# uibk-uncover/ws-unet

Measured on AMD Instinct MI355X. Metric: 512x512 grayscale images/sec (UNet predict), higher is better.
Workload: dtype f16 MFMA on the f16 halves + ONE block-scaled fp4 (e2m1) MFMA per tap pair for both residual cross terms (per-pixel / per-(co, tap) E8M0 scales), fp32 accumulate; planar storage

## Files before the change

### ws_unet_amd/csrc/conv3x3_qu.hip

```cpp
#include "wsu_device.h"

namespace {

constexpr int TW = 32, TH = 16;
constexpr int CW = 17, CH = 9, CPIX = CW * CH;
constexpr int NPIX_S = 4 * CPIX;
constexpr int PLANE_S = NPIX_S * 16;
constexpr int SEG_S = (NPIX_S + 63) / 64;
constexpr int IN_S = 3 * PLANE_S + SEG_S * 256;
constexpr int LP = 33, LH = TH / 2 + 2, LW_ = TW / 2 + 2;
constexpr int NPIX_L = LP * LH;
constexpr int PLANE_L = NPIX_L * 16;
constexpr int SEG_L = (NPIX_L + 63) / 64;
constexpr int IN_L = 3 * PLANE_L + SEG_L * 256;
constexpr int W_GRAN_S = 9 * 3 * WSU_COB * 16;
constexpr int W_S = W_GRAN_S + 1024;
constexpr int W_UNITS_L = 8;
constexpr int W_GRAN_L = W_UNITS_L * 3 * WSU_COB * 16;
constexpr int W_L = W_GRAN_L + 1024;
constexpr int PIECES_S = W_S / 1024, PIECES_L = W_L / 1024;
constexpr int REGION = 80640;
constexpr int OFF_SW = IN_S, OFF_LIN = W_L, OFF_LW1 = W_L + IN_L;
constexpr int LDS_BIAS = 2 * REGION;
constexpr int MAX_COUT = 512;
constexpr int LDS_TOTAL = LDS_BIAS + MAX_COUT * 4;
static_assert(IN_S + W_S <= REGION && OFF_LW1 + W_L <= REGION && (REGION & 0xF) == 0 && LDS_TOTAL <= 160 * 1024, "LDS budget");
static_assert((OFF_SW | OFF_LIN | OFF_LW1) % 16 == 0, "16-byte aligned allocations");
constexpr int ZERO_BYTES = 576;
constexpr int LDS_ZERO = 2 * REGION - ZERO_BYTES;
static_assert(IN_S + W_S <= REGION - ZERO_BYTES && OFF_LW1 + W_L <= REGION - ZERO_BYTES && LDS_ZERO % 16 == 0 && ZERO_BYTES >= 2 * CW * 16 + 16 + 16, "zero block");
constexpr int NLOAD = 4, NWAVE = 8, NT = (NWAVE + NLOAD) * 64;
constexpr unsigned OOB = 0xFFFFFFF0u;
constexpr int W_S_H = 9 * 2 * WSU_COB * 16;
constexpr int W_L_H = W_UNITS_L * 2 * WSU_COB * 16;
constexpr int PIECES_S_H = W_S_H / 1024, PIECES_L_H = W_L_H / 1024;

struct UArgs {
    const char* xl; const char* xs; const char* wps; const char* wpl; const float* bias;
    char* y;
    int n, h, w, hl, wl, cl, c2, cout;
    int tiles_x, tiles_y, ltiles_x, ncb, nchS, nchL;
    int relu, ntiles;
    unsigned* range_flag;
};

struct Tile { int n, y0, x0, cb; };
__device__ __forceinline__ Tile tile_of(const UArgs& a, int t) {
    Tile r;
    r.cb = t % a.ncb; t /= a.ncb;
    const int tx = t % a.tiles_x; t /= a.tiles_x;
    const int ty = t % a.tiles_y;
    r.n = t / a.tiles_y; r.y0 = ty * TH; r.x0 = tx * TW;
    return r;
}

typedef __attribute__((address_space(3))) void lds_void;
typedef __attribute__((address_space(3))) char lds_char;

__device__ __forceinline__ void wait_vm(int n) {
#define WSU_VM_CASE(k) case k: asm volatile("s_waitcnt vmcnt(" #k ")" ::: "memory"); break;
    switch (n) {
        WSU_VM_CASE(0) WSU_VM_CASE(1) WSU_VM_CASE(2) WSU_VM_CASE(3) WSU_VM_CASE(4) WSU_VM_CASE(5) WSU_VM_CASE(6) WSU_VM_CASE(7) WSU_VM_CASE(8) WSU_VM_CASE(9)
        WSU_VM_CASE(10) WSU_VM_CASE(11) WSU_VM_CASE(12) WSU_VM_CASE(13) WSU_VM_CASE(14) WSU_VM_CASE(15) WSU_VM_CASE(16) WSU_VM_CASE(17) WSU_VM_CASE(18) WSU_VM_CASE(19)
        WSU_VM_CASE(20) WSU_VM_CASE(21) WSU_VM_CASE(22) WSU_VM_CASE(23) WSU_VM_CASE(24) WSU_VM_CASE(25) WSU_VM_CASE(26) WSU_VM_CASE(27) WSU_VM_CASE(28) WSU_VM_CASE(29)
        WSU_VM_CASE(30) WSU_VM_CASE(31) WSU_VM_CASE(32) WSU_VM_CASE(33) WSU_VM_CASE(34) WSU_VM_CASE(35) WSU_VM_CASE(36) WSU_VM_CASE(37) WSU_VM_CASE(38) WSU_VM_CASE(39)
        default: asm volatile("s_waitcnt vmcnt(0)" ::: "memory"); break;
    }
#undef WSU_VM_CASE
}


template <int FMT, int LW>
__device__ __forceinline__ void u_loader(const UArgs& a, char* smem, int lane, int lw, int G, int K) {
    constexpr bool H = FMT == WSU_PLANAR_H;
    constexpr int NSS = LW < 2 ? 3 : 2;
    constexpr int NSL = LW < 2 ? 2 : 1;
    constexpr int OPS_INS = (H ? 2 : 4) * NSS, OPS_INL = (H ? 2 : 4) * NSL;
    constexpr int WS0 = H ? (LW < 2 ? LW * 3 : 6 + (LW - 2) * 6) : (LW < 2 ? LW * 5 : 10 + (LW - 2) * 9);
    constexpr int NWS = H ? (LW < 2 ? 3 : 6) : (LW < 2 ? 5 : 9);
    constexpr int WL0 = H ? (LW < 2 ? LW * 3 : 6 + (LW - 2) * 5) : (LW < 2 ? LW * 5 : (LW == 2 ? 10 : 17));
    constexpr int NWL = H ? (LW < 2 ? 3 : 5) : (LW < 2 ? 5 : (LW == 2 ? 7 : 8));
    constexpr int WSLICE_S = H ? W_S_H : W_S, WSLICE_L = H ? W_L_H : W_L;
    static_assert(2 * 5 + 2 * 9 == PIECES_S && 2 * 5 + 7 + 8 == PIECES_L, "weight pieces over the loader waves");
    static_assert(2 * 3 + 2 * 6 == PIECES_S_H && 2 * 3 + 2 * 5 == PIECES_L_H, "weight pieces over the loader waves (format H)");
    lds_char* smem3 = (lds_char*)smem;
    const unsigned hw16 = (unsigned)(a.h * a.w) * 16u, hwl16 = (unsigned)(a.hl * a.wl) * 16u;
    const unsigned cbytes_s = H ? (unsigned)wsu_h_chunk_bytes(a.h, a.w) : (unsigned)wsu_q_chunk_bytes(a.h, a.w);
    const unsigned cbytes_l = H ? (unsigned)wsu_h_chunk_bytes(a.hl, a.wl) : (unsigned)wsu_q_chunk_bytes(a.hl, a.wl);
    const int T = a.nchS + a.nchL;
    const int J = K * T;
    if (J <= 0) return;
    unsigned voS[NSS], soS[NSS], voL[NSL], soL[NSL];
    auto plan = [&](const Tile& t) __attribute__((always_inline)) {
        WSU_STATIC_FOR(NSS, k, {
            const int idx = min((LW + NLOAD * k) * 64 + lane, NPIX_S - 1);
            const int p = idx / CPIX, rem = idx - p * CPIX;
            const int lr = rem / CW, lc = rem - lr * CW;
            const int yy = wsu_reflect(t.y0 - 1 + 2 * lr + (p >> 1), a.h), xx = wsu_reflect(t.x0 - 1 + 2 * lc + (p & 1), a.w);
            voS[k] = (unsigned)(yy * a.w + xx) * 16u;
            if constexpr (!H) soS[k] = 3u * hw16 + wsu_q_soff(yy, xx, a.tiles_x);
        });
        WSU_STATIC_FOR(NSL, k, {
            const int idx = min((LW + NLOAD * k) * 64 + lane, NPIX_L - 1);
            const int r = idx / LP, c = min(idx - r * LP, LW_ - 1);
            const int yy = min(max((t.y0 >> 1) - 1 + r, 0), a.hl - 1), xx = min(max((t.x0 >> 1) - 1 + c, 0), a.wl - 1);
            voL[k] = (unsigned)(yy * a.wl + xx) * 16u;
            if constexpr (!H) soL[k] = 3u * hwl16 + wsu_q_soff(yy, xx, a.ltiles_x);
        });
    };
    int a_kt = 0, a_c = 0, a_r = 0; bool a_low = false;
    Tile at = tile_of(a, lw);
    unsigned region = 0;
    auto issue_alloc = [&](lds_char* slot) __attribute__((always_inline)) {
        int nops;
        const bool is_in = a_low ? a_r == 1 : a_r == 0;
        if (is_in && !a_low) {
            const char* src = a.xs + ((size_t)at.n * a.nchS + a_c) * cbytes_s;
            const auto rs = __builtin_amdgcn_make_buffer_rsrc(const_cast<char*>(src), 0, (int)cbytes_s, 0x00020000);
            WSU_STATIC_FOR(NSS, k, {
                constexpr int seg = LW + NLOAD * k;
                if (seg < SEG_S - 1 || lane < NPIX_S - (SEG_S - 1) * 64) {
                    __builtin_amdgcn_raw_ptr_buffer_load_lds(rs, (lds_void*)(slot + seg * 1024), 16, voS[k], 0, 0, 0);
                    __builtin_amdgcn_raw_ptr_buffer_load_lds(rs, (lds_void*)(slot + PLANE_S + seg * 1024), 16, voS[k], (int)hw16, 0, 0);
                    if constexpr (!H) {
                        __builtin_amdgcn_raw_ptr_buffer_load_lds(rs, (lds_void*)(slot + 2 * PLANE_S + seg * 1024), 16, voS[k], (int)(2u * hw16), 0, 0);
                        __builtin_amdgcn_raw_ptr_buffer_load_lds(rs, (lds_void*)(slot + 3 * PLANE_S + seg * 256), 1, soS[k], 0, 0, 0);
                    }
                }
            });
            nops = OPS_INS;
        } else if (is_in) {
            const char* src = a.xl + ((size_t)at.n * a.nchL + a_c) * cbytes_l;
            const auto rs = __builtin_amdgcn_make_buffer_rsrc(const_cast<char*>(src), 0, (int)cbytes_l, 0x00020000);
            WSU_STATIC_FOR(NSL, k, {
                constexpr int seg = LW + NLOAD * k;
                if (seg < SEG_L - 1 || lane < NPIX_L - (SEG_L - 1) * 64) {
                    __builtin_amdgcn_raw_ptr_buffer_load_lds(rs, (lds_void*)(slot + seg * 1024), 16, voL[k], 0, 0, 0);
                    __builtin_amdgcn_raw_ptr_buffer_load_lds(rs, (lds_void*)(slot + PLANE_L + seg * 1024), 16, voL[k], (int)hwl16, 0, 0);
                    if constexpr (!H) {
                        __builtin_amdgcn_raw_ptr_buffer_load_lds(rs, (lds_void*)(slot + 2 * PLANE_L + seg * 1024), 16, voL[k], (int)(2u * hwl16), 0, 0);
                        __builtin_amdgcn_raw_ptr_buffer_load_lds(rs, (lds_void*)(slot + 3 * PLANE_L + seg * 256), 1, soL[k], 0, 0, 0);
                    }
                }
            });
            nops = OPS_INL;
        } else if (!a_low) {
            const auto rs = __builtin_amdgcn_make_buffer_rsrc(const_cast<char*>(a.wps), 0, 0x7FFFFFF0, 0x00020000);
            const int base = (at.cb * a.nchS + a_c) * WSLICE_S;
            WSU_STATIC_FOR(NWS, k, {
                constexpr int piece = WS0 + k;
                __builtin_amdgcn_raw_ptr_buffer_load_lds(rs, (lds_void*)(slot + piece * 1024), 16, (unsigned)lane * 16u, base + piece * 1024, 0, 0);
            });
            nops = NWS;
        } else {
            const auto rs = __builtin_amdgcn_make_buffer_rsrc(const_cast<char*>(a.wpl), 0, 0x7FFFFFF0, 0x00020000);
            const int base = ((at.cb * a.nchL + a_c) * 2 + (a_r == 2 ? 1 : 0)) * WSLICE_L;
            WSU_STATIC_FOR(NWL, k, {
                constexpr int piece = WL0 + k;
                __builtin_amdgcn_raw_ptr_buffer_load_lds(rs, (lds_void*)(slot + piece * 1024), 16, (unsigned)lane * 16u, base + piece * 1024, 0, 0);
            });
            nops = NWL;
        }
        return nops;
    };
    auto issue_step = [&]() __attribute__((always_inline)) {
        lds_char* base = smem3 + region;
        int nops;
        if (!a_low) {
            a_r = 0; nops = issue_alloc(base);
            a_r = 1; nops += issue_alloc(base + OFF_SW);
            if (++a_c == a.nchS) { a_c = 0; a_low = true; }
        } else {
            a_r = 0; nops = issue_alloc(base);
            a_r = 1; nops += issue_alloc(base + OFF_LIN);
            a_r = 2; nops += issue_alloc(base + OFF_LW1);
            if (++a_c == a.nchL) {
                a_low = false; a_c = 0;
                if (++a_kt < K) { at = tile_of(a, lw + a_kt * G); plan(at); }
            }
        }
        region ^= (unsigned)REGION;
        return nops;
    };
    plan(at);
    {
        issue_step();
        const int n1 = J > 1 ? issue_step() : 0;
        wait_vm(n1);
    }
    for (int j = 0; ; ++j) {
        __builtin_amdgcn_s_barrier();
        asm volatile("" ::: "memory");
        if (j + 1 >= J) break;
        if (j >= 1) issue_step();
        wait_vm(0);
    }
}

template <int FMT>
__global__ __launch_bounds__(NT) __attribute__((amdgpu_waves_per_eu(3, 3)))
void conv3x3_qu_kernel(const UArgs a) {
    constexpr bool H = FMT == WSU_PLANAR_H;
    constexpr int WPL = H ? 2 : 3;
    extern __shared__ __attribute__((aligned(16))) char smem[];
    const int tid = threadIdx.x;
    const int wv = __builtin_amdgcn_readfirstlane(tid >> 6), lane = tid & 63;
    const int G = gridDim.x;
    const int lw = (int)wsu_xcd_remap(blockIdx.x, G);
    const int K = a.ntiles > lw ? (a.ntiles - lw + G - 1) / G : 0;
    float* s_bias = reinterpret_cast<float*>(smem + LDS_BIAS);
    for (int i = tid; i < a.cout; i += NT) s_bias[i] = a.bias ? a.bias[i] : 0.f;
    if constexpr (!H) {
        for (int i = tid; i < ZERO_BYTES / 4; i += NT) reinterpret_cast<unsigned*>(smem + LDS_ZERO)[i] = 0u;
        asm volatile("s_waitcnt lgkmcnt(0)" ::: "memory");
    }

    if (wv >= NWAVE) {
        switch (wv - NWAVE) {
            case 0: u_loader<FMT, 0>(a, smem, lane, lw, G, K); break;
            case 1: u_loader<FMT, 1>(a, smem, lane, lw, G, K); break;
            case 2: u_loader<FMT, 2>(a, smem, lane, lw, G, K); break;
            default: u_loader<FMT, 3>(a, smem, lane, lw, G, K); break;
        }
        return;
    }

    const int cls = wv & 3, py = cls >> 1, px = cls & 1, rh = wv >> 2;
    const int l31 = lane & 31, hh = lane >> 5;
    const int lrow = l31 >> 4, lcol = lrow ? ((l31 + 15) & 15) : l31;
    const unsigned laneS = (unsigned)(((4 * rh + lrow) * CW + lcol) * 16), laneL = (unsigned)(((4 * rh + lrow) * LP + lcol) * 16);
    constexpr unsigned QS = 2 * CW * 16, QL = 2 * LP * 16;
    Tile cur = tile_of(a, lw);
    f32x16 acc[2][2];
    unsigned region = 0;
    unsigned in_off = 0, w_off = 0;
    auto next_region = [&]() __attribute__((always_inline)) { const unsigned r = region; region ^= (unsigned)REGION; return r; };
    int hh_q = hh;
    typedef __attribute__((address_space(3))) const unsigned char lds_cuchar;
    typedef __attribute__((address_space(3))) const int lds_cint;
    typedef __attribute__((address_space(3))) const u32x4 lds_cu32x4;
    lds_char* L = (lds_char*)smem;
    const unsigned Lb = (unsigned)(size_t)L;
    auto at = [](unsigned addr) __attribute__((always_inline)) { return (lds_char*)(size_t)addr; };
    auto tap_s = [&](int ky, int kx) __attribute__((always_inline)) {
        return (unsigned)(((((py + ky) & 1) * 2 + ((px + kx) & 1)) * CPIX + ((py + ky) >> 1) * CW + ((px + kx) >> 1)) * 16);
    };
    unsigned a_off = 0, b_off = 0, hd_w = 0, hd_sa = 0, hd_b = 0, hd_sb = 0, x_w = 0, x_w4 = 0, x_sa = 0, x_sa4 = 0, x_b4 = 0;
    constexpr unsigned W4_IMM = (unsigned)((8 * 3 + 2) * 64) * 16u;
    unsigned tap_sel[5] = {};
    if constexpr (!H) {
        WSU_STATIC_FOR(5, tp, {
            constexpr int t0 = 2 * tp, t1 = (2 * tp + 1 < 9) ? 2 * tp + 1 : 2 * tp;
            tap_sel[tp] = ((hh ? tap_s(t1 / 3, t1 % 3) : tap_s(t0 / 3, t0 % 3)) + laneS) >> 2;
            asm volatile("" : "+v"(tap_sel[tp]));
        });
    }
    auto sync_step = [&](auto low_c) __attribute__((always_inline)) {
        constexpr bool LOW = decltype(low_c)::value;
        const unsigned r = next_region();
        in_off = LOW ? r + OFF_LIN : r;
        w_off = LOW ? r : r + OFF_SW;
        hh_q = hh;
        asm volatile("" : "+v"(hh_q));
        a_off = Lb + w_off + (unsigned)l31 * 16u + (unsigned)hh * 1024u;
        b_off = Lb + in_off + (unsigned)hh * (LOW ? PLANE_L : PLANE_S) + (LOW ? laneL : laneS);
        if constexpr (!H && !LOW) {
            const unsigned hq = (unsigned)hh_q, zero = Lb + (unsigned)LDS_ZERO;
            const unsigned w0 = Lb + w_off + (unsigned)l31 * 16u;
            x_w = w0 + hq * (unsigned)(3 * 64 * 16);
            x_w4 = hq ? zero - W4_IMM : w0;
            x_sa4 = Lb + w_off + W_GRAN_S + (unsigned)l31;
            x_sa = x_sa4 + hq * 64u;
            hd_b = Lb + in_off + 2 * PLANE_S + tap_sel[0] * 4u;
            hd_sb = Lb + in_off + 3 * PLANE_S + tap_sel[0];
            x_b4 = hq ? zero : Lb + in_off + 2 * PLANE_S + tap_sel[4] * 4u;
            asm volatile("" : "+v"(a_off), "+v"(b_off), "+v"(x_w), "+v"(x_w4), "+v"(x_sa), "+v"(x_sa4), "+v"(hd_b), "+v"(hd_sb), "+v"(x_b4));
        } else if constexpr (!H) {
            const int u = cls * 2 + hh_q;
            const unsigned pb = (unsigned)((py * LP + px) * 16) + (unsigned)hh_q * 16u + laneL;
            hd_w = Lb + w_off + (unsigned)((u * 3 + 2) * 64 + l31) * 16u;
            hd_sa = Lb + w_off + W_GRAN_L + (unsigned)(u * 64 + l31);
            hd_b = Lb + in_off + 2 * PLANE_L + pb;
            hd_sb = Lb + in_off + 3 * PLANE_L + (pb >> 2);
            asm volatile("" : "+v"(a_off), "+v"(b_off), "+v"(hd_w), "+v"(hd_sa), "+v"(hd_b), "+v"(hd_sb));
        } else {
            asm volatile("" : "+v"(a_off), "+v"(b_off));
        }
        __builtin_amdgcn_s_barrier();
        asm volatile("" ::: "memory");
    };
    struct Frag { u32x4 a[2]; u32x4 b[2]; int sa[2]; int sb[2]; };
    auto load_unit = [&](auto u_c, Frag& f) __attribute__((always_inline)) {
        constexpr int u = decltype(u_c)::value, tp = u / 3, k = u % 3;
        if constexpr (k == 0) {
            constexpr bool single = 2 * tp + 1 >= 9;
            constexpr unsigned wimm = (unsigned)((6 * tp + 2) * 64) * 16u;
            static_assert(!single || wimm == W4_IMM, "tap 8");
            const unsigned wb = single ? x_w4 : x_w, sab = single ? x_sa4 : x_sa;
            const unsigned bb = tp == 0 ? hd_b : (single ? x_b4 : Lb + in_off + 2 * PLANE_S + tap_sel[tp] * 4u);
            const unsigned sbb = tp == 0 ? hd_sb : Lb + in_off + 3 * PLANE_S + tap_sel[tp];
_Pragma("unroll")
            for (int m = 0; m < 2; ++m) { f.a[m] = *(lds_cu32x4*)(at(wb) + wimm + m * 512); f.sa[m] = *(lds_cuchar*)(at(sab) + 128 * tp + m * 32); }
_Pragma("unroll")
            for (int q = 0; q < 2; ++q) {
                f.b[q] = *(lds_cu32x4*)(at(bb) + q * QS);
                f.sb[q] = *(lds_cint*)(at(sbb) + q * (QS >> 2));
            }
        } else {
            constexpr int tap = 2 * tp + k - 1;
            const unsigned pb = b_off + tap_s(tap / 3, tap % 3);
_Pragma("unroll")
            for (int m = 0; m < 2; ++m) f.a[m] = *(lds_cu32x4*)(at(a_off) + ((tap * WPL) * 64) * 16 + m * 512);
_Pragma("unroll")
            for (int q = 0; q < 2; ++q) f.b[q] = *(lds_cu32x4*)(at(pb) + q * QS);
        }
    };
    auto mma_unit = [&](auto u_c, Frag& f, auto first_c) __attribute__((always_inline)) {
        constexpr int u = decltype(u_c)::value, k = u % 3;
        constexpr bool FIRST = decltype(first_c)::value && u == 0;
_Pragma("unroll")
        for (int m = 0; m < 2; ++m)
_Pragma("unroll")
            for (int q = 0; q < 2; ++q) {
                if constexpr (k != 0) wsu_mfma_f16(f.a[m], f.b[q], acc[m][q]);
                else if constexpr (FIRST) acc[m][q] = wsu_mfma_q4_z(f.a[m], f.b[q], f.sa[m], f.sb[q]);
                else wsu_mfma_q4(f.a[m], f.b[q], f.sa[m], f.sb[q], acc[m][q]);
            }
    };
    auto skip_units = [&](auto first_c) __attribute__((always_inline)) {
        constexpr bool FIRST = decltype(first_c)::value;
        if constexpr (!H) {
            constexpr int NU = 14;
            Frag fr[2];
            load_unit(std::integral_constant<int, 0>{}, fr[0]);
            WSU_STATIC_FOR(NU, u, {
                if constexpr (u + 1 < NU) load_unit(std::integral_constant<int, u + 1>{}, fr[(u + 1) % 2]);
                __builtin_amdgcn_sched_barrier(0);
                mma_unit(u_c, fr[u % 2], first_c);
                __builtin_amdgcn_sched_barrier(0);
            });
        } else {
            WSU_STATIC_FOR(9, tap, {
                u32x4 ah[2], bh[2];
                const unsigned pb = b_off + tap_s(tap / 3, tap % 3);
_Pragma("unroll")
                for (int m = 0; m < 2; ++m) ah[m] = *(lds_cu32x4*)(at(a_off) + ((tap * WPL) * 64) * 16 + m * 512);
_Pragma("unroll")
                for (int q = 0; q < 2; ++q) bh[q] = *(lds_cu32x4*)(at(pb) + q * QS);
_Pragma("unroll")
                for (int m = 0; m < 2; ++m)
_Pragma("unroll")
                    for (int q = 0; q < 2; ++q) {
                        if constexpr (FIRST && tap == 0) acc[m][q] = wsu_mfma_f16_z(ah[m], bh[q]);
                        else wsu_mfma_f16(ah[m], bh[q], acc[m][q]);
                    }
            });
        }
    };
    auto low_units = [&](auto dy_c) __attribute__((always_inline)) {
        constexpr int dy = decltype(dy_c)::value;
        constexpr unsigned WDY = dy ? (unsigned)(OFF_LW1) : 0u;
        const unsigned rowo = (unsigned)(((py + dy) * LP + px) * 16);
        if constexpr (!H) {
            const int u = cls * 2 + hh_q;
            u32x4 a4[2], b4[2]; int sa[2], sb[2];
            const unsigned pb = rowo + (unsigned)hh_q * 16u + laneL;
            const unsigned wb = dy == 0 ? hd_w : Lb + w_off + WDY + (unsigned)((u * 3 + 2) * 64 + l31) * 16u;
            const unsigned sab = dy == 0 ? hd_sa : Lb + w_off + WDY + W_GRAN_L + (unsigned)(u * 64 + l31);
            const unsigned bb = dy == 0 ? hd_b : Lb + in_off + 2 * PLANE_L + pb;
            const unsigned sbb = dy == 0 ? hd_sb : Lb + in_off + 3 * PLANE_L + (pb >> 2);
_Pragma("unroll")
            for (int m = 0; m < 2; ++m) { a4[m] = *(lds_cu32x4*)(at(wb) + m * 512); sa[m] = *(lds_cuchar*)(at(sab) + m * 32); }
_Pragma("unroll")
            for (int q = 0; q < 2; ++q) {
                b4[q] = *(lds_cu32x4*)(at(bb) + q * QL);
                sb[q] = *(lds_cint*)(at(sbb) + q * (QL >> 2));
            }
_Pragma("unroll")
            for (int m = 0; m < 2; ++m)
_Pragma("unroll")
                for (int q = 0; q < 2; ++q) wsu_mfma_q4(a4[m], b4[q], sa[m], sb[q], acc[m][q]);
        }
        WSU_STATIC_FOR(2, dx, {
            u32x4 ah[2], bh[2];
            const unsigned wb = a_off + WDY + (unsigned)(((cls * 2 + dx) * WPL) * 64) * 16u;
            const unsigned pb = b_off + rowo + dx * 16u;
_Pragma("unroll")
            for (int m = 0; m < 2; ++m) ah[m] = *(lds_cu32x4*)(at(wb) + m * 512);
_Pragma("unroll")
            for (int q = 0; q < 2; ++q) bh[q] = *(lds_cu32x4*)(at(pb) + q * QL);
_Pragma("unroll")
            for (int m = 0; m < 2; ++m)
_Pragma("unroll")
                for (int q = 0; q < 2; ++q) wsu_mfma_f16(ah[m], bh[q], acc[m][q]);
        });
    };

    auto finish_tile = [&]() __attribute__((always_inline)) {
        int l31o = l31, hho = hh, lro = lrow, lco = lcol;
        asm volatile("" : "+v"(l31o), "+v"(hho), "+v"(lro), "+v"(lco));
        const unsigned hw16 = (unsigned)(a.h * a.w) * 16u;
        const unsigned cbytes = (unsigned)wsu_q_chunk_bytes(a.h, a.w);
        const int nco = a.cout >> 4;
        const int X = cur.x0 + 2 * lco + px;
        const int Y0 = cur.y0 + 2 * (4 * rh + lro) + py, Y1 = Y0 + 4;
        const bool ok0 = Y0 < a.h && X < a.w, ok1 = Y1 < a.h && X < a.w;
        const unsigned off0 = (unsigned)(Y0 * a.w + X) * 16u, off1 = (unsigned)(Y1 * a.w + X) * 16u;
        const unsigned so0 = wsu_q_soff(Y0, X, a.tiles_x), so1 = wsu_q_soff(Y1, X, a.tiles_x);
        const unsigned hpl = hho ? hw16 : 0u;
        const bool okm = hho ? ok1 : ok0;
        unsigned og0 = ok0 ? off0 + hpl : OOB, og1 = ok1 ? off1 + hpl : OOB;
        unsigned oq = okm ? (hho ? off1 : off0) + 2u * hw16 : OOB, os = okm ? 3u * hw16 + (hho ? so1 : so0) : OOB;
        asm volatile("" : "+v"(og0), "+v"(og1), "+v"(oq), "+v"(os));
        const float relu_floor = a.relu ? 0.f : -__builtin_inff();
        float vmax = 0.f;
        WSU_STATIC_FOR(2, m, {
            WSU_STATIC_FOR(2, cp, {
                const int oc = cur.cb * 4 + m * 2 + cp;
                const int co0 = oc * 16 + 4 * hho;
                const f32x4 bx = *reinterpret_cast<const f32x4*>(s_bias + co0), by = *reinterpret_cast<const f32x4*>(s_bias + co0 + 8);
                f32x4 vx[2], vy[2];
_Pragma("unroll")
                for (int q = 0; q < 2; ++q)
_Pragma("unroll")
                    for (int e = 0; e < 4; ++e) {
                        const float x = fmaxf(acc[m][q][8 * cp + e] + bx[e], relu_floor), y = fmaxf(acc[m][q][8 * cp + 4 + e] + by[e], relu_floor);
                        vx[q][e] = x; vy[q][e] = y;
                        if constexpr (H) vmax = fmaxf(fmaxf(vmax, fabsf(x)), fabsf(y));
                    }
                if constexpr (H) {
                    char* base = a.y + ((size_t)cur.n * nco + oc) * (2u * hw16);
                    const auto rs = __builtin_amdgcn_make_buffer_rsrc(base, 0, (int)(2u * hw16), 0x00020000);
                    __builtin_amdgcn_raw_buffer_store_b128(wsu_h_granule(vx[0], vy[0]), rs, (int)og0, 0, 0);
                    __builtin_amdgcn_raw_buffer_store_b128(wsu_h_granule(vx[1], vy[1]), rs, (int)og1, 0, 0);
                    return;
                }
                u32x4 g0, g1; uint32_t dh0, dr0, sb0, dh1, dr1, sb1;
                const float mx0 = wsu_q4_pre(vx[0], vy[0], g0, dh0, dr0, sb0);
                const float mx1 = wsu_q4_pre(vx[1], vy[1], g1, dh1, dr1, sb1);
                vmax = wsu_max3(vmax, mx0, mx1);
                const u32x4 qg = wsu_q4_pair(dh0, dr0, dh1, dr1);
                char* base = a.y + ((size_t)cur.n * nco + oc) * cbytes;
                const auto rs = __builtin_amdgcn_make_buffer_rsrc(base, 0, (int)cbytes, 0x00020000);
                __builtin_amdgcn_raw_buffer_store_b128(g0, rs, (int)og0, 0, 0);
                __builtin_amdgcn_raw_buffer_store_b128(g1, rs, (int)og1, 0, 0);
                __builtin_amdgcn_raw_buffer_store_b128(qg, rs, (int)oq, 0, 0);
                __builtin_amdgcn_raw_buffer_store_b8((unsigned char)(hho ? sb1 : sb0), rs, (int)os, 0, 0);
            });
        });
        if (a.range_flag && __builtin_amdgcn_ballot_w64(!(vmax <= (H ? WSU_F16_RANGE : WSU_F8_RANGE))) != 0 && lane == 0) atomicOr(a.range_flag, 1u);
    };

    for (int t = 0; t < K; ++t) {
        sync_step(std::false_type{});
        skip_units(std::true_type{});
        for (int c = 1; c < a.nchS; ++c) {
            sync_step(std::false_type{});
            skip_units(std::false_type{});
        }
        for (int c = 0; c < a.nchL; ++c) {
            sync_step(std::true_type{});
            low_units(std::integral_constant<int, 0>{});
            low_units(std::integral_constant<int, 1>{});
        }
        finish_tile();
        if (t + 1 < K) cur = tile_of(a, lw + (t + 1) * G);
    }
}

template <int FMT>
__global__ void pack_up_low_kernel(const float* __restrict__ w3, const float* __restrict__ wt, char* __restrict__ dst, float* __restrict__ wc_dense,
                                   int cup, int c2, int cl, int cout) {
    const int nchL = cl / 16, ctot = cup + c2;
    const long long total = (long long)(cout / WSU_COB) * nchL * 2 * W_UNITS_L * WSU_COB;
    for (long long d = (long long)blockIdx.x * blockDim.x + threadIdx.x; d < total; d += (long long)gridDim.x * blockDim.x) {
        long long t = d;
        const int co = (int)(t % WSU_COB); t /= WSU_COB;
        const int u = (int)(t % W_UNITS_L); t /= W_UNITS_L;
        const int dy = (int)(t & 1); t >>= 1;
        const int c = (int)(t % nchL); const int cb = (int)(t / nchL);
        const int cls = u >> 1, dx = u & 1, py = cls >> 1, px = cls & 1;
        const int ky0 = py == 0 ? (dy == 0 ? 0 : 1) : (dy == 0 ? 0 : 2), ky1 = py == 0 ? (dy == 0 ? 0 : 2) : (dy == 0 ? 1 : 2);
        const int kx0 = px == 0 ? (dx == 0 ? 0 : 1) : (dx == 0 ? 0 : 2), kx1 = px == 0 ? (dx == 0 ? 0 : 2) : (dx == 0 ? 1 : 2);
        const int cog = cb * WSU_COB + co;
        float v[16], r[16];
#pragma unroll
        for (int e = 0; e < 16; ++e) v[e] = 0.f;
        for (int ci = 0; ci < cup; ++ci)
            for (int ky = ky0; ky <= ky1; ++ky)
                for (int kx = kx0; kx <= kx1; ++kx) {
                    const float w = w3[(((size_t)cog * ctot + ci) * 3 + ky) * 3 + kx];
                    const int sy = (py + ky + 1) & 1, sx = (px + kx + 1) & 1;
#pragma unroll
                    for (int e = 0; e < 16; ++e) v[e] = fmaf(w, wt[(((size_t)(c * 16 + e) * cup + ci) * 2 + sy) * 2 + sx], v[e]);
                }
        if (wc_dense)
#pragma unroll
            for (int e = 0; e < 16; ++e) wc_dense[((((size_t)cog * cl + c * 16 + e) * 2 + py) * 2 + px) * 4 + dy * 2 + dx] = v[e];
        uint32_t h[8];
#pragma unroll
        for (int e = 0; e < 8; ++e) {
            const _Float16 x = (_Float16)v[2 * e], y = (_Float16)v[2 * e + 1];
            h[e] = (uint32_t)__builtin_bit_cast(unsigned short, x) | ((uint32_t)__builtin_bit_cast(unsigned short, y) << 16);
            r[2 * e] = (v[2 * e] - (float)x) * 2048.f; r[2 * e + 1] = (v[2 * e + 1] - (float)y) * 2048.f;
        }
        const u32x4 h0 = mk_u4(h[0], h[1], h[2], h[3]), h1 = mk_u4(h[4], h[5], h[6], h[7]);
        if constexpr (FMT == WSU_PLANAR_H) {
            char* base = dst + (((size_t)cb * nchL + c) * 2 + dy) * W_L_H + (size_t)(u * 2) * (WSU_COB * 16) + co * 16;
            *reinterpret_cast<u32x4*>(base) = h0;
            *reinterpret_cast<u32x4*>(base + WSU_COB * 16) = h1;
            continue;
        }
        const int E = wsu_q4_block_exp(wsu_f16x16_max_abs_bits(h0, h1));
        const float sc = wsu_pow2f(E);
        uint32_t q[4] = {0, 0, 0, 0};
        WSU_STATIC_FOR(8, e, { q[e >> 2] = __builtin_amdgcn_cvt_scalef32_pk_fp4_f32(q[e >> 2], r[2 * e], r[2 * e + 1], sc, e & 3); });
        q[2] = wsu_f16x8_to_fp4(h0, sc); q[3] = wsu_f16x8_to_fp4(h1, sc);
        char* slice = dst + (((size_t)cb * nchL + c) * 2 + dy) * W_L;
        char* base = slice + (size_t)(u * 3) * (WSU_COB * 16) + co * 16;
        *reinterpret_cast<u32x4*>(base) = h0;
        *reinterpret_cast<u32x4*>(base + WSU_COB * 16) = h1;
        *reinterpret_cast<u32x4*>(base + 2 * WSU_COB * 16) = mk_u4(q[0], q[1], q[2], q[3]);
        slice[W_GRAN_L + u * 64 + co] = (char)(E + 127 - 11);
        if (u == 0 && co < 32) *reinterpret_cast<u32x4*>(slice + W_GRAN_L + 512 + co * 16) = mk_u4(0, 0, 0, 0);
    }
}

__global__ void up_bias_kernel(const float* __restrict__ w3, const float* __restrict__ bt, const float* __restrict__ b3, float* __restrict__ out, int cup, int c2, int cout) {
    const int co = blockIdx.x * blockDim.x + threadIdx.x;
    if (co >= cout) return;
    float s = b3 ? b3[co] : 0.f;
    if (bt)
        for (int ci = 0; ci < cup; ++ci) {
            float t = 0.f;
            for (int k = 0; k < 9; ++k) t += w3[((size_t)co * (cup + c2) + ci) * 9 + k];
            s = fmaf(bt[ci], t, s);
        }
    out[co] = s;
}

struct UFormat {
    const char* pack; const char* fwd;
    void (*pack_kernel)(const float*, const float*, char*, float*, int, int, int, int); const char* pack_kernel_name;
    void (*kernel)(const UArgs); const char* kernel_name; const char* lds_name;
    int w_s, w_l;
};
const UFormat& u_format(int fmt) {
    static const UFormat q = {"conv3x3_up_pack", "conv3x3_up_q", pack_up_low_kernel<WSU_PLANAR_Q>, "pack_up_low_kernel",
                              conv3x3_qu_kernel<WSU_PLANAR_Q>, "conv3x3_qu_kernel", "conv3x3_qu", W_S, W_L};
    static const UFormat h = {"conv3x3_up_pack_h", "conv3x3_up_h", pack_up_low_kernel<WSU_PLANAR_H>, "pack_up_low_kernel<H>",
                              conv3x3_qu_kernel<WSU_PLANAR_H>, "conv3x3_qu_kernel<H>", "conv3x3_qu<H>", W_S_H, W_L_H};
    return fmt == WSU_PLANAR_H ? h : q;
}

size_t up_packed_bytes(int fmt, int cl, int cout) {
    if (cl <= 0 || cout <= 0 || cl % 16 || cout % WSU_COB) return 0;
    return (size_t)(cout / WSU_COB) * (cl / 16) * 2 * u_format(fmt).w_l;
}

int up_pack(int fmt, const float* w3_oihw, const float* wt, const float* bt, const float* b3, void* w_low_packed, float* bias_out, float* wc_dense,
            int cl, int cup, int c2, int cout, void* stream) {
    const UFormat& f = u_format(fmt);
    WSU_REQUIRE(w3_oihw && wt && w_low_packed && bias_out, "%s: null pointer", f.pack);
    WSU_REQUIRE(cl > 0 && cl % 16 == 0 && cup > 0 && c2 >= 0 && cout > 0 && cout % WSU_COB == 0,
                "%s: cl=%d must be a multiple of 16, cout=%d of %d, cup=%d > 0", f.pack, cl, cout, WSU_COB, cup);
    hipStream_t s = static_cast<hipStream_t>(stream);
    hipLaunchKernelGGL(f.pack_kernel, dim3(1024), dim3(128), 0, s, w3_oihw, wt, (char*)w_low_packed, wc_dense, cup, c2, cl, cout);
    int rc = wsu_check_launch(f.pack_kernel_name);
    if (rc != WSU_OK) return rc;
    hipLaunchKernelGGL(up_bias_kernel, dim3((cout + 63) / 64), dim3(64), 0, s, w3_oihw, bt, b3, bias_out, cup, c2, cout);
    return wsu_check_launch("up_bias_kernel");
}

int up_fwd(int fmt, const void* x_low, const void* x_skip, const void* w_skip_packed, const void* w_low_packed, const float* bias, void* y,
           int n, int h, int w, int cl, int c2, int cout, int relu, unsigned* range_flag, void* stream) {
    const UFormat& f = u_format(fmt);
    const char* who = f.fwd;
    WSU_REQUIRE(x_low && x_skip && w_skip_packed && w_low_packed && y, "%s: null pointer", who);
    WSU_REQUIRE(n > 0 && h >= 2 && w >= 2 && h % 2 == 0 && w % 2 == 0, "%s: bad shape n=%d h=%d w=%d (the output of a stride-2 transposed conv is even)", who, n, h, w);
    WSU_REQUIRE(cl > 0 && cl % 16 == 0 && c2 > 0 && c2 % 16 == 0, "%s: cl=%d c2=%d must be positive multiples of 16", who, cl, c2);
    WSU_REQUIRE(cout > 0 && cout % WSU_COB == 0 && cout <= MAX_COUT, "%s: cout=%d must be a multiple of %d (<= %d)", who, cout, WSU_COB, MAX_COUT);
    WSU_REQUIRE((long long)h * w * 50 < 0xFFFFFFF0LL, "%s: h*w too large (a chunk must stay below 4 GiB)", who);
    UArgs a;
    a.xl = (const char*)x_low; a.xs = (const char*)x_skip; a.wps = (const char*)w_skip_packed; a.wpl = (const char*)w_low_packed; a.bias = bias;
    a.y = (char*)y;
    a.n = n; a.h = h; a.w = w; a.hl = h / 2; a.wl = w / 2; a.cl = cl; a.c2 = c2; a.cout = cout;
    a.tiles_x = (w + TW - 1) / TW; a.tiles_y = (h + TH - 1) / TH; a.ltiles_x = (a.wl + 31) / 32; a.ncb = cout / WSU_COB;
    a.nchS = c2 / 16; a.nchL = cl / 16; a.relu = relu; a.range_flag = range_flag;
    const long long nt = (long long)n * a.tiles_x * a.tiles_y * a.ncb;
    WSU_REQUIRE(nt > 0 && nt < 0x3FFFFFFFLL, "%s: %lld tiles out of range", who, nt);
    WSU_REQUIRE((long long)a.ncb * a.nchL * 2 * f.w_l < 0x7FFFFFF0LL && (long long)a.ncb * a.nchS * f.w_s < 0x7FFFFFF0LL, "%s: packed weights beyond 2 GiB", who);
    a.ntiles = (int)nt;
    const int ncu = wsu_cu_count(who);
    if (!ncu) return WSU_ERR_HIP;
    static bool raised[2] = {false, false};
    bool& done = raised[fmt == WSU_PLANAR_H];
    if (!done) {
        if (int rc = wsu_raise_lds(f.kernel, LDS_TOTAL, f.lds_name)) return rc;
        done = true;
    }
    hipLaunchKernelGGL(f.kernel, dim3(a.ntiles < ncu ? a.ntiles : ncu), dim3(NT), LDS_TOTAL, static_cast<hipStream_t>(stream), a);
    return wsu_check_launch(f.kernel_name);
}

}

extern "C" {

size_t wsu_conv3x3_up_packed_bytes(int cl, int cout) { return up_packed_bytes(WSU_PLANAR_Q, cl, cout); }

int wsu_conv3x3_up_pack(const float* w3_oihw, const float* wt, const float* bt, const float* b3, void* w_low_packed, float* bias_out, float* wc_dense,
                        int cl, int cup, int c2, int cout, void* stream) {
    return up_pack(WSU_PLANAR_Q, w3_oihw, wt, bt, b3, w_low_packed, bias_out, wc_dense, cl, cup, c2, cout, stream);
}

int wsu_conv3x3_up_q_fwd(const void* x_low, const void* x_skip, const void* w_skip_packed, const void* w_low_packed, const float* bias, void* y,
                         int n, int h, int w, int cl, int c2, int cout, int relu, unsigned* range_flag, void* stream) {
    return up_fwd(WSU_PLANAR_Q, x_low, x_skip, w_skip_packed, w_low_packed, bias, y, n, h, w, cl, c2, cout, relu, range_flag, stream);
}

size_t wsu_conv3x3_up_packed_h_bytes(int cl, int cout) { return up_packed_bytes(WSU_PLANAR_H, cl, cout); }

int wsu_conv3x3_up_pack_h(const float* w3_oihw, const float* wt, const float* bt, const float* b3, void* w_low_packed, float* bias_out, float* wc_dense,
                          int cl, int cup, int c2, int cout, void* stream) {
    return up_pack(WSU_PLANAR_H, w3_oihw, wt, bt, b3, w_low_packed, bias_out, wc_dense, cl, cup, c2, cout, stream);
}

int wsu_conv3x3_up_h_fwd(const void* x_low, const void* x_skip, const void* w_skip_packed, const void* w_low_packed, const float* bias, void* y,
                         int n, int h, int w, int cl, int c2, int cout, int relu, unsigned* range_flag, void* stream) {
    return up_fwd(WSU_PLANAR_H, x_low, x_skip, w_skip_packed, w_low_packed, bias, y, n, h, w, cl, c2, cout, relu, range_flag, stream);
}

}
```

Baseline: 3862.

## Store low-res tile rows split by parity to cut padding and DMA segments

Changes the LDS layout of the low-resolution input tile. Rows are now split into an even block and an odd block, with the odd block at offset 97, which replaces the earlier padded 33-pixel row pitch. This shrinks the tile so it fits in three DMA segments that each loader wave issues at most once, and the weight pieces are redistributed evenly across the loader waves. The offset of 97 keeps adjacent rows one granule apart mod 16, which is meant to avoid LDS bank conflicts. In exchange, per-lane address setup now needs two row bases (b_off, b_off1), which adds live registers.

```diff
diff --git a/ws_unet_amd/csrc/conv3x3_qu.hip b/ws_unet_amd/csrc/conv3x3_qu.hip
--- a/ws_unet_amd/csrc/conv3x3_qu.hip
+++ b/ws_unet_amd/csrc/conv3x3_qu.hip
@@ -8,11 +8,13 @@
 constexpr int PLANE_S = NPIX_S * 16;
 constexpr int SEG_S = (NPIX_S + 63) / 64;
 constexpr int IN_S = 3 * PLANE_S + SEG_S * 256;
-constexpr int LP = 33, LH = TH / 2 + 2, LW_ = TW / 2 + 2;
-constexpr int NPIX_L = LP * LH;
+constexpr int LH = TH / 2 + 2, LW_ = TW / 2 + 2;
+constexpr int LEVEN = (LH + 1) / 2 * LW_, LODD = 97;
+constexpr int NPIX_L = LODD + LH / 2 * LW_;
 constexpr int PLANE_L = NPIX_L * 16;
 constexpr int SEG_L = (NPIX_L + 63) / 64;
 constexpr int IN_L = 3 * PLANE_L + SEG_L * 256;
+static_assert(LODD >= LEVEN && (LODD - 1) % 16 == 0 && (LODD - LW_ + 1) % 16 == 0 && NPIX_L <= 192, "low tile: adjacent rows one granule apart mod 16, three DMA segments");
 constexpr int W_GRAN_S = 9 * 3 * WSU_COB * 16;
 constexpr int W_S = W_GRAN_S + 1024;
 constexpr int W_UNITS_L = 8;
@@ -74,15 +76,16 @@
 __device__ __forceinline__ void u_loader(const UArgs& a, char* smem, int lane, int lw, int G, int K) {
     constexpr bool H = FMT == WSU_PLANAR_H;
     constexpr int NSS = LW < 2 ? 3 : 2;
-    constexpr int NSL = LW < 2 ? 2 : 1;
+    constexpr int NSL = LW < SEG_L ? 1 : 0;
     constexpr int OPS_INS = (H ? 2 : 4) * NSS, OPS_INL = (H ? 2 : 4) * NSL;
     constexpr int WS0 = H ? (LW < 2 ? LW * 3 : 6 + (LW - 2) * 6) : (LW < 2 ? LW * 5 : 10 + (LW - 2) * 9);
     constexpr int NWS = H ? (LW < 2 ? 3 : 6) : (LW < 2 ? 5 : 9);
-    constexpr int WL0 = H ? (LW < 2 ? LW * 3 : 6 + (LW - 2) * 5) : (LW < 2 ? LW * 5 : (LW == 2 ? 10 : 17));
-    constexpr int NWL = H ? (LW < 2 ? 3 : 5) : (LW < 2 ? 5 : (LW == 2 ? 7 : 8));
+    constexpr int WL0 = H ? LW * 4 : LW * 6;
+    constexpr int NWL = H ? 4 : (LW < 3 ? 6 : 7);
     constexpr int WSLICE_S = H ? W_S_H : W_S, WSLICE_L = H ? W_L_H : W_L;
-    static_assert(2 * 5 + 2 * 9 == PIECES_S && 2 * 5 + 7 + 8 == PIECES_L, "weight pieces over the loader waves");
-    static_assert(2 * 3 + 2 * 6 == PIECES_S_H && 2 * 3 + 2 * 5 == PIECES_L_H, "weight pieces over the loader waves (format H)");
+    static_assert(2 * 5 + 2 * 9 == PIECES_S && 3 * 6 + 7 == PIECES_L, "weight pieces over the loader waves");
+    static_assert(2 * 3 + 2 * 6 == PIECES_S_H && 4 * 4 == PIECES_L_H, "weight pieces over the loader waves (format H)");
+    static_assert(SEG_L <= NLOAD && OPS_INL + 2 * NWL <= (H ? 10 : 16), "a low step's pieces per loader wave");
     lds_char* smem3 = (lds_char*)smem;
     const unsigned hw16 = (unsigned)(a.h * a.w) * 16u, hwl16 = (unsigned)(a.hl * a.wl) * 16u;
     const unsigned cbytes_s = H ? (unsigned)wsu_h_chunk_bytes(a.h, a.w) : (unsigned)wsu_q_chunk_bytes(a.h, a.w);
@@ -90,7 +93,7 @@
     const int T = a.nchS + a.nchL;
     const int J = K * T;
     if (J <= 0) return;
-    unsigned voS[NSS], soS[NSS], voL[NSL], soL[NSL];
+    unsigned voS[NSS], soS[NSS], voL[1], soL[1];
     auto plan = [&](const Tile& t) __attribute__((always_inline)) {
         WSU_STATIC_FOR(NSS, k, {
             const int idx = min((LW + NLOAD * k) * 64 + lane, NPIX_S - 1);
@@ -102,7 +105,8 @@
         });
         WSU_STATIC_FOR(NSL, k, {
             const int idx = min((LW + NLOAD * k) * 64 + lane, NPIX_L - 1);
-            const int r = idx / LP, c = min(idx - r * LP, LW_ - 1);
+            const int odd = idx >= LODD ? 1 : 0, e = min(idx - odd * LODD, LEVEN - 1);
+            const int r2 = e / LW_, r = 2 * r2 + odd, c = e - r2 * LW_;
             const int yy = min(max((t.y0 >> 1) - 1 + r, 0), a.hl - 1), xx = min(max((t.x0 >> 1) - 1 + c, 0), a.wl - 1);
             voL[k] = (unsigned)(yy * a.wl + xx) * 16u;
             if constexpr (!H) soL[k] = 3u * hwl16 + wsu_q_soff(yy, xx, a.ltiles_x);
@@ -228,8 +232,10 @@
     const int cls = wv & 3, py = cls >> 1, px = cls & 1, rh = wv >> 2;
     const int l31 = lane & 31, hh = lane >> 5;
     const int lrow = l31 >> 4, lcol = lrow ? ((l31 + 15) & 15) : l31;
-    const unsigned laneS = (unsigned)(((4 * rh + lrow) * CW + lcol) * 16), laneL = (unsigned)(((4 * rh + lrow) * LP + lcol) * 16);
-    constexpr unsigned QS = 2 * CW * 16, QL = 2 * LP * 16;
+    const unsigned laneS = (unsigned)(((4 * rh + lrow) * CW + lcol) * 16);
+    auto low_lane = [&](int s) __attribute__((always_inline)) { return (unsigned)(((2 * rh + (s >> 1)) * LW_ + (s & 1) * LODD + lcol + px) * 16); };
+    const unsigned laneL0 = low_lane(py + lrow), laneL1 = low_lane(py + 1 + lrow);
+    constexpr unsigned QS = 2 * CW * 16, QL = LW_ * 16;
     Tile cur = tile_of(a, lw);
     f32x16 acc[2][2];
     unsigned region = 0;
@@ -245,7 +251,7 @@
     auto tap_s = [&](int ky, int kx) __attribute__((always_inline)) {
         return (unsigned)(((((py + ky) & 1) * 2 + ((px + kx) & 1)) * CPIX + ((py + ky) >> 1) * CW + ((px + kx) >> 1)) * 16);
     };
-    unsigned a_off = 0, b_off = 0, hd_w = 0, hd_sa = 0, hd_b = 0, hd_sb = 0, x_w = 0, x_w4 = 0, x_sa = 0, x_sa4 = 0, x_b4 = 0;
+    unsigned a_off = 0, b_off = 0, b_off1 = 0, hd_w = 0, hd_sa = 0, hd_b = 0, hd_sb = 0, x_w = 0, x_w4 = 0, x_sa = 0, x_sa4 = 0, x_b4 = 0;
     constexpr unsigned W4_IMM = (unsigned)((8 * 3 + 2) * 64) * 16u;
     unsigned tap_sel[5] = {};
     if constexpr (!H) {
@@ -263,7 +269,8 @@
         hh_q = hh;
         asm volatile("" : "+v"(hh_q));
         a_off = Lb + w_off + (unsigned)l31 * 16u + (unsigned)hh * 1024u;
-        b_off = Lb + in_off + (unsigned)hh * (LOW ? PLANE_L : PLANE_S) + (LOW ? laneL : laneS);
+        b_off = Lb + in_off + (unsigned)hh * (LOW ? PLANE_L : PLANE_S) + (LOW ? laneL0 : laneS);
+        if constexpr (LOW) b_off1 = b_off - laneL0 + laneL1;
         if constexpr (!H && !LOW) {
             const unsigned hq = (unsigned)hh_q, zero = Lb + (unsigned)LDS_ZERO;
             const unsigned w0 = Lb + w_off + (unsigned)l31 * 16u;
@@ -277,12 +284,14 @@
             asm volatile("" : "+v"(a_off), "+v"(b_off), "+v"(x_w), "+v"(x_w4), "+v"(x_sa), "+v"(x_sa4), "+v"(hd_b), "+v"(hd_sb), "+v"(x_b4));
         } else if constexpr (!H) {
             const int u = cls * 2 + hh_q;
-            const unsigned pb = (unsigned)((py * LP + px) * 16) + (unsigned)hh_q * 16u + laneL;
+            const unsigned pb = (unsigned)hh_q * 16u + laneL0;
             hd_w = Lb + w_off + (unsigned)((u * 3 + 2) * 64 + l31) * 16u;
             hd_sa = Lb + w_off + W_GRAN_L + (unsigned)(u * 64 + l31);
             hd_b = Lb + in_off + 2 * PLANE_L + pb;
             hd_sb = Lb + in_off + 3 * PLANE_L + (pb >> 2);
-            asm volatile("" : "+v"(a_off), "+v"(b_off), "+v"(hd_w), "+v"(hd_sa), "+v"(hd_b), "+v"(hd_sb));
+            asm volatile("" : "+v"(a_off), "+v"(b_off), "+v"(b_off1), "+v"(hd_w), "+v"(hd_sa), "+v"(hd_b), "+v"(hd_sb));
+        } else if constexpr (LOW) {
+            asm volatile("" : "+v"(a_off), "+v"(b_off), "+v"(b_off1));
         } else {
             asm volatile("" : "+v"(a_off), "+v"(b_off));
         }
@@ -360,11 +369,10 @@
     auto low_units = [&](auto dy_c) __attribute__((always_inline)) {
         constexpr int dy = decltype(dy_c)::value;
         constexpr unsigned WDY = dy ? (unsigned)(OFF_LW1) : 0u;
-        const unsigned rowo = (unsigned)(((py + dy) * LP + px) * 16);
         if constexpr (!H) {
             const int u = cls * 2 + hh_q;
             u32x4 a4[2], b4[2]; int sa[2], sb[2];
-            const unsigned pb = rowo + (unsigned)hh_q * 16u + laneL;
+            const unsigned pb = (unsigned)hh_q * 16u + (dy ? laneL1 : laneL0);
             const unsigned wb = dy == 0 ? hd_w : Lb + w_off + WDY + (unsigned)((u * 3 + 2) * 64 + l31) * 16u;
             const unsigned sab = dy == 0 ? hd_sa : Lb + w_off + WDY + W_GRAN_L + (unsigned)(u * 64 + l31);
             const unsigned bb = dy == 0 ? hd_b : Lb + in_off + 2 * PLANE_L + pb;
@@ -384,7 +392,7 @@
         WSU_STATIC_FOR(2, dx, {
             u32x4 ah[2], bh[2];
             const unsigned wb = a_off + WDY + (unsigned)(((cls * 2 + dx) * WPL) * 64) * 16u;
-            const unsigned pb = b_off + rowo + dx * 16u;
+            const unsigned pb = (dy ? b_off1 : b_off) + dx * 16u;
 _Pragma("unroll")
             for (int m = 0; m < 2; ++m) ah[m] = *(lds_cu32x4*)(at(wb) + m * 512);
 _Pragma("unroll")
```

New measurement: 3873, median of 6. Within noise of the previous version (+0.3%).
